# manuelbb-upb/Morbit.jl

Hardware: AMD Instinct MI355X
Metric: RBF build+solve+eval cycles/sec (higher is better)
Workload: dtype f64

## Files before the change

### include/mrbf.h

```cpp
#ifndef MRBF_H
#define MRBF_H

#include <stdint.h>

#ifdef __cplusplus
extern "C" {
#endif

typedef struct mrbf_ctx mrbf_ctx;
typedef struct mrbf_model mrbf_model;

enum {
    MRBF_CUBIC = 0,
    MRBF_INV_MULTIQUADRIC = 1,
    MRBF_MULTIQUADRIC = 2,
    MRBF_THIN_PLATE_SPLINE = 3,
    MRBF_GAUSSIAN = 4
};

enum {
    MRBF_OK = 0,
    MRBF_ENOTPD = 1,
    MRBF_ESINGULAR = 2,
    MRBF_EHIP = 3,
// ... 161 lines not shown
    const double *centres, *values;
    double *weights_out, *poly_out;
    mrbf_model *model;
    int32_t status;
    int32_t reserved;
    mrbf_fit_info info;
} mrbf_fit_job;
int32_t mrbf_fit_batch(mrbf_ctx *ctx, int64_t n_starts, mrbf_fit_job *jobs, float *ms_total);

int32_t mrbf_debug_env(const char *name);
int32_t mrbf_debug_mfma_layout(mrbf_ctx *ctx, double *out16x16_a_times_b, const double *A16x4, const double *B4x16);
int32_t mrbf_debug_potrf(mrbf_ctx *ctx, int64_t n, double *A_colmajor_inout, int32_t impl, int32_t *info, float *ms);
int32_t mrbf_debug_diag(mrbf_ctx *ctx, const double *A128, int32_t reps, float *ms_per_call, double *shader_cycles,
                        double *realtime_us);
int32_t mrbf_debug_mfma_peak(mrbf_ctx *ctx, int32_t blocks_per_cu, int32_t threads, int32_t iters, float *ms, double *tflops);
int32_t mrbf_debug_mfma_asm(mrbf_ctx *ctx, int32_t variant, int32_t blocks_per_cu, int32_t iters, float *ms, double *tflops,
                            double *cycles_per_mfma);
int32_t mrbf_debug_dgemm(mrbf_ctx *ctx, int32_t m, int32_t n, int32_t k, float *ms, double *tflops);
int32_t mrbf_debug_mega_tables(int32_t nt, int32_t mt, int32_t slack, int32_t slack_chain, int32_t first, int32_t win, int32_t srows,
                               int32_t half_cols, int64_t *out6);
int32_t mrbf_debug_mega_tables2(int32_t nt, int32_t mt, int32_t slack, int32_t slack_chain, int32_t first, int32_t win, int32_t srows,
                                int32_t half_cols, const int32_t *opt5, int64_t *out6);
int32_t mrbf_debug_mega_plan(int32_t nt, int32_t mt, int32_t xreal, int64_t *out39);

enum { MRBF_PS_OK = 0, MRBF_PS_CRITICAL = 1, MRBF_PS_FAILURE = 2 };
typedef struct {
    int32_t max_ideal_evals;
    int32_t max_ps_evals;
    int32_t max_polish_evals;
    int32_t reserved;
    uint64_t seed;
    double t0;
    double xtol_rel;
} mrbf_ps_options;
typedef struct {
    int32_t status;
    int32_t generations;
    int32_t evals_ideal, evals_ps, evals_polish;
    float ms_total;
    double tau;
} mrbf_ps_info;
int32_t mrbf_ps_step(mrbf_ctx *ctx, const mrbf_model *model, const double *x_n, const double *lb_eff, const double *ub_eff,
                     const double *fx_n, const double *r_or_null, const mrbf_ps_options *opts, double *x_trial, double *mx_trial,
                     double *r_out, mrbf_ps_info *info);

enum { MRBF_ROLE_NONE = -1, MRBF_ROLE_EQ = -2, MRBF_ROLE_INEQ = -3 };
// ... 120 lines not shown
```

### morbit.jl_amd/_lib.py

```python
import ctypes
import os

import numpy as np

_HERE = os.path.dirname(os.path.abspath(__file__))
LIB_PATH = os.environ.get("MRBF_LIB") or os.path.join(_HERE, "libmrbf.so")

c_dp = ctypes.POINTER(ctypes.c_double)
c_fp = ctypes.POINTER(ctypes.c_float)
c_ip = ctypes.POINTER(ctypes.c_int32)
c_vp = ctypes.c_void_p

MRBF_OK, MRBF_ENOTPD, MRBF_ESINGULAR, MRBF_EHIP, MRBF_EBLAS, MRBF_ENOMEM, MRBF_ENODEVICE, MRBF_ENCCL = range(8)
PATH_CHOL, PATH_PROJ_CHOL, PATH_LU, PATH_MINNORM, PATH_ROUND4 = 1, 2, 3, 4, 5
OPT_GRAM_MODE, OPT_RESIDUAL, OPT_FORCE_PATH, OPT_CHOL_IMPL, OPT_EVAL_IMPL, OPT_TIMING, OPT_DIAG_IMPL, OPT_CHOL_WINDOW = 1, 2, 3, 4, 5, 6, 7, 8
OPT_SPIN_MS, OPT_DEBUG_FAULT, OPT_LAST_DEVICE_MS, OPT_SLOW_LAUNCHES = 9, 10, 11, 12
OPT_ARENA_BYTES, OPT_LIVE_HANDLES = 13, 14
FB_CHOL_HOST_DRIVEN, FB_BACKSOLVE_BLOCKED, FB_LU = 1, 2, 4


class FitInfo(ctypes.Structure):
    _fields_ = [("path", ctypes.c_int32), ("factor_info", ctypes.c_int32), ("n", ctypes.c_int32), ("q", ctypes.c_int32),
                ("rel_residual", ctypes.c_double), ("max_pitw", ctypes.c_double), ("mu", ctypes.c_double),
                ("ms_gram", ctypes.c_float), ("ms_project", ctypes.c_float), ("ms_factor", ctypes.c_float),
# ... 158 lines not shown
                                     ctypes.c_double, ctypes.c_int32, ctypes.c_int32, ctypes.c_double, c_vp, c_ip, ctypes.POINTER(c_vp)]),
    "mrbf_fit_from_round4": (ctypes.c_int32, [c_vp, c_vp, ctypes.c_int32, c_vp, ctypes.POINTER(c_vp), c_vp, c_vp, ctypes.POINTER(FitInfo)]),
    "mrbf_round4_sites": (ctypes.c_int32, [c_vp, ctypes.POINTER(ctypes.c_int64), ctypes.POINTER(ctypes.c_int64), c_ip]),
    "mrbf_free_round4": (ctypes.c_int32, [c_vp, c_vp]),
    "mrbf_round4_batch": (ctypes.c_int32, [c_vp, ctypes.c_int64, ctypes.c_int32, ctypes.POINTER(Round4Job), c_fp]),
    "mrbf_dispatch_round4_batch": (ctypes.c_int32, [ctypes.c_int64, ctypes.c_int32]),
    "mrbf_model_dims": (ctypes.c_int32, [c_vp, ctypes.POINTER(ctypes.c_int64), c_ip, c_ip, c_ip]),
    "mrbf_free_model": (ctypes.c_int32, [c_vp, c_vp]),
    "mrbf_batch_run": (ctypes.c_int32, [ctypes.c_int32, c_ip, ctypes.c_int64, ctypes.POINTER(Problem),
                                        ctypes.POINTER(Result)]),
    "mrbf_fit_batch": (ctypes.c_int32, [c_vp, ctypes.c_int64, ctypes.POINTER(FitJob), c_fp]),
    "mrbf_dispatch_fit_batch": (ctypes.c_int32, [ctypes.c_int64]),
    "mrbf_debug_mfma_layout": (ctypes.c_int32, [c_vp, c_vp, c_vp, c_vp]),
    "mrbf_debug_potrf": (ctypes.c_int32, [c_vp, ctypes.c_int64, c_vp, ctypes.c_int32, c_ip, c_fp]),
    "mrbf_debug_env": (ctypes.c_int32, [ctypes.c_char_p]),
    "mrbf_debug_diag": (ctypes.c_int32, [c_vp, c_vp, ctypes.c_int32, c_fp, c_dp, c_dp]),
    "mrbf_debug_ps_rank": (ctypes.c_int32, [c_vp, ctypes.c_int32, c_vp, c_vp, ctypes.c_uint64, ctypes.c_int32, ctypes.c_int32, c_ip, c_ip]),
    "mrbf_debug_mfma_peak": (ctypes.c_int32, [c_vp, ctypes.c_int32, ctypes.c_int32, ctypes.c_int32, c_fp, c_dp]),
    "mrbf_debug_mfma_asm": (ctypes.c_int32, [c_vp, ctypes.c_int32, ctypes.c_int32, ctypes.c_int32, c_fp, c_dp, c_dp]),
    "mrbf_debug_dgemm": (ctypes.c_int32, [c_vp, ctypes.c_int32, ctypes.c_int32, ctypes.c_int32, c_fp, c_dp]),
    "mrbf_debug_mega_tables": (ctypes.c_int32, [ctypes.c_int32] * 8 + [c_vp]),
    "mrbf_debug_mega_tables2": (ctypes.c_int32, [ctypes.c_int32] * 8 + [c_vp, c_vp]),
    "mrbf_debug_mega_plan": (ctypes.c_int32, [ctypes.c_int32] * 3 + [c_vp]),
    "mrbf_stochastic_rank": (ctypes.c_int32, [ctypes.c_int32, c_vp, c_vp, c_vp, ctypes.c_double, c_vp]),
    "mrbf_ps_step": (ctypes.c_int32, [c_vp, c_vp, c_vp, c_vp, c_vp, c_vp, c_vp, ctypes.POINTER(PsOptions), c_vp, c_vp, c_vp,
                                      ctypes.POINTER(PsInfo)]),
    "mrbf_ps_step_problem": (ctypes.c_int32, [c_vp, ctypes.POINTER(PsProblem), c_vp, c_vp, c_vp, c_vp, c_vp, ctypes.POINTER(PsOptions),
                                              c_vp, c_vp, c_vp, ctypes.POINTER(PsInfo)]),
    "mrbf_sd_direction": (ctypes.c_int32, [c_vp, ctypes.c_int64, ctypes.c_int32, ctypes.c_int32, ctypes.c_int32, ctypes.c_int32] + [c_vp] * 8
                          + [ctypes.c_int32, c_vp, c_vp, c_vp, c_vp, c_vp]),
    "mrbf_sd_criticality": (ctypes.c_int32, [c_vp, ctypes.POINTER(PsProblem), c_vp, c_vp, c_vp, c_vp, ctypes.c_int32, c_vp, c_vp,
                                             ctypes.POINTER(SdInfo)]),
    "mrbf_normal_direction": (ctypes.c_int32, [c_vp, ctypes.c_int64, ctypes.c_int32, ctypes.c_int32, ctypes.c_int32] + [c_vp] * 12),
    "mrbf_normal_step": (ctypes.c_int32, [c_vp, ctypes.POINTER(PsProblem), ctypes.c_int32, c_vp, c_vp, c_vp, ctypes.c_double, ctypes.c_double,
                                          ctypes.c_double, ctypes.c_int32, c_vp, c_vp, ctypes.POINTER(NormalInfo)]),
    "mrbf_sd_step": (ctypes.c_int32, [c_vp, ctypes.POINTER(PsProblem), c_vp, c_vp, ctypes.c_double, c_vp, c_vp, ctypes.c_double, c_vp,
                                      ctypes.POINTER(SdStepOptions), c_vp, c_vp, ctypes.POINTER(SdStepInfo)]),
    "mrbf_sd_iterate_batch": (ctypes.c_int32, [c_vp, ctypes.c_int64, ctypes.POINTER(PsProblem), ctypes.POINTER(ctypes.c_void_p), c_vp, c_vp, c_vp,
                                               c_vp, c_vp, ctypes.c_int32, ctypes.POINTER(SdStepOptions), c_vp, c_vp, c_vp,
                                               ctypes.POINTER(SdBatchRecord), c_fp]),
    "mrbf_dispatch_sd_batch": (ctypes.c_int32, [ctypes.c_int64] + [ctypes.c_int32] * 7),
    "mrbf_normal_step_batch": (ctypes.c_int32, [c_vp, ctypes.c_int64, ctypes.POINTER(PsProblem), ctypes.POINTER(ctypes.c_void_p), ctypes.c_int32,
                                                c_vp, c_vp, c_vp, c_vp, ctypes.c_double, ctypes.c_double, ctypes.c_int32, c_vp, c_vp, c_vp,
                                                ctypes.POINTER(NormalBatchRecord), c_fp]),
    "mrbf_dispatch_normal_batch": (ctypes.c_int32, [ctypes.c_int64] + [ctypes.c_int32] * 5),
    "mrbf_dispatch_ps": (ctypes.c_int32, [ctypes.c_int32] * 6),
# ... 100 lines not shown
```

### morbit.jl_amd/csrc/chol_mega.hip

```cpp
#include <chrono>

#include "chol_diag_core.hpp"
#include "common.hpp"
#include "mega_gemm.hpp"

namespace mrbf {

typedef double v4d __attribute__((ext_vector_type(4)));
typedef double v2d __attribute__((ext_vector_type(2)));

namespace mega {

constexpr int WIN_DEFAULT = 4;

enum { JOB_U = 0, JOB_T = 1, JOB_P = 2, JOB_S = 3, JOB_UH = 4 };
struct Job {
    short kind, i, c, w;
};
enum { CTL_QP = 0, CTL_ABORT = 32, CTL_TIMEOUT = 64, CTL_PCOLS = 96, CTL_QC = 128, CTL_TS = 144 , CTL_WORDS = 160 };
constexpr int QSTRIDE = 32;
__host__ __device__ inline int wstart(int w, int first, int win) { return w <= 0 ? 0 : first + win * (w - 1); }
__host__ __device__ inline int nbulk_updates(int i, int c, int slack, int slack_chain, int first, int win, int srows = 2) {
    const int t = c - ((i - c <= srows) ? slack_chain : slack);
    return t < first ? 0 : (t - first) / win + 1;
// ... 24 lines not shown
    unsigned *sprog;
    unsigned *quiet;
    int nwin;
    int *info;
    const Job *cjobs;
    int nchainjobs;
    int nchain;
    int ndedicated;
    int look;
    unsigned long long spin_ticks;
    int fault;
    int use_quiet;
    int xchain;
    int quiet_tail;
    int slack, slack_chain, first, win, wbias, srows;
    Edge edge;
    int cboost;
    int head_job1;
    int nreserve;
    int reserve_job0;
    unsigned long long *jlog;
    int jlog_cap;
    int pstream;
    int panel_dma;
    int trace_dbg;
    unsigned long long *trace;
};

struct Shared {
    union {
        double gemm[4 * 2 * 8 * LDS_LD];
        diagcore::DiagV6Shared diag;
    } u;
    int ok;
    int jkind, jidx;
    unsigned long long *jrec;
    int wlo;
    int cwlo;
    int mycu;
};

typedef __attribute__((address_space(1))) unsigned gu32;
typedef __attribute__((address_space(1))) double gf64;
__device__ __forceinline__ unsigned ldf(const unsigned *p) {
    return __hip_atomic_load((const gu32 *)p, __ATOMIC_RELAXED, __HIP_MEMORY_SCOPE_AGENT);
}
// ... 155 lines not shown
                }
            }
        }
    }
}

template <int TM>
__device__ __forceinline__ void load_tile_neg(const double *__restrict__ C, int64_t ldc, v4d (&acc)[TM / 32][4]) {
    constexpr int NJ = TM / 32;
    const int lane = threadIdx.x & 63, wave = threadIdx.x >> 6;
    const int l15 = lane & 15, l4 = lane >> 4;
    const int ioff = (TM == 128) ? (wave >> 1) * 64 : 0;
    const int joff = (TM == 128) ? (wave & 1) * 64 : wave * 32;
#pragma unroll
    for (int j = 0; j < NJ; ++j)
#pragma unroll
        for (int r = 0; r < 4; ++r) {
            const int64_t gj = joff + j * 16 + l4 + 4 * r;
#pragma unroll
            for (int i = 0; i < 4; ++i) acc[j][i][r] = -*(const gf64 *)&C[(ioff + i * 16 + l15) + gj * ldc];
        }
}

#define JLOG(k)                                                             \
    do {                                                                   \
        if (sh.jrec && threadIdx.x == 0) sh.jrec[k] = wall_clock64();      \
    } while (0)

template <int TM>
__device__ __attribute__((noinline)) bool run_bulk(const Args &a, Shared &sh, const Job jb) {
    const int64_t lda = uni64(a.lda);
    double *const A = uni_ptr(a.A);
    const int i = __builtin_amdgcn_readfirstlane(jb.i), c = __builtin_amdgcn_readfirstlane(jb.c), jw = __builtin_amdgcn_readfirstlane(jb.w);
    const int w = jw & 255, hcode = jw >> 8, roff = (TM == 64 && hcode == 1) ? 64 : 0;
    const int pl = wstart(w + 1, a.first, a.win) - 1;
    if (!wg_wait(sh, a, a.tdone + (size_t)i * a.NT + pl, 2u, a.tdone + (size_t)c * a.NT + pl, 2u, a.ucnt + (size_t)i * a.NT + c,
                 (unsigned)(2 * w), 0x100u))
        return false;
    JLOG(2);
    v4d acc[TM / 32][4];
    double *C = A + (int64_t)i * NB + roff + (int64_t)c * NB * lda;
    load_tile_neg<TM>(C, lda, acc);
    const int64_t k0 = (int64_t)wstart(w, a.first, a.win) * NB;
    gemm_acc<TM>(A + (int64_t)i * NB + roff + k0 * lda, lda, A + (int64_t)c * NB + k0 * lda, lda,
                 (wstart(w + 1, a.first, a.win) - wstart(w, a.first, a.win)) * NB, acc, sh.u.gemm);
    JLOG(3);
#pragma unroll
    for (int j = 0; j < TM / 32; ++j)
#pragma unroll
        for (int i2 = 0; i2 < 4; ++i2) acc[j][i2] = -acc[j][i2];
    if (i == c)
        store_tile<TM, false, true, true>(C, lda, acc, roff);
    else
        store_tile<TM, false, false, true>(C, lda, acc);
    wg_drain();
    if (threadIdx.x == 0) addf(a.ucnt + (size_t)i * a.NT + c, (TM == 128 || hcode == 2) ? 2u : 1u);
    return true;
}

template <int TM>
__device__ __forceinline__ bool window_part(const Args &a, Shared &sh, int i, int c, int pend, int roff,
                                                      unsigned long long *tr) {
    const int64_t lda = uni64(a.lda);
    double *const A = uni_ptr(a.A);
    const int wc = nbulk_updates(i, c, a.slack, a.slack_chain, a.first, a.win, srows_at(c, a.srows, a.edge)), p0 = wstart(wc, a.first, a.win);
    const unsigned *uc = a.ucnt + (size_t)i * a.NT + c;
    if (p0 >= pend) return wg_wait(sh, a, uc, (unsigned)(2 * wc), nullptr, 0, nullptr, 0, 0x200u);
    v4d acc[TM / 32][4];
    zero_acc(acc);
    for (int p = p0; p < pend;) {
        if (threadIdx.x == 0) {
            bool ok = poll_ge(a.tdone + (size_t)i * a.NT + p, 2u, a, 0x210u) && poll_ge(a.tdone + (size_t)c * a.NT + p, 2u, a, 0x211u);
            int run = 0;
            if (ok) {
                run = 1;
                while (p + run < pend && ldf(a.tdone + (size_t)i * a.NT + p + run) >= 2u && ldf(a.tdone + (size_t)c * a.NT + p + run) >= 2u) ++run;
            }
            __builtin_amdgcn_fence(__ATOMIC_ACQUIRE, "agent");
            asm volatile("s_waitcnt vmcnt(0)" ::: "memory");
            sh.ok = run;
        }
        __syncthreads();
        const int run = sh.ok;
        __syncthreads();
        if (run == 0) return false;
        if (tr && threadIdx.x == 0) tr[p == p0 ? 5 : 6] = wall_clock64();
        JLOG(p == p0 ? 2 : 3);
        const int64_t k0 = (int64_t)p * NB;
        gemm_acc<TM>(A + (int64_t)i * NB + roff + k0 * lda, lda, A + (int64_t)c * NB + k0 * lda, lda, run * NB, acc, sh.u.gemm);
        p += run;
    }
    if (tr && threadIdx.x == 0) tr[7] = wall_clock64();
    if (!wg_wait(sh, a, uc, (unsigned)(2 * wc), nullptr, 0, nullptr, 0, 0x212u)) return false;
    double *C = A + (int64_t)i * NB + roff + (int64_t)c * NB * lda;
    if (TM == 128 && i == c)
        store_tile<TM, true, true, false>(C, lda, acc);
    else
        store_tile<TM, true, false, false>(C, lda, acc);
    asm volatile("s_waitcnt vmcnt(0)" ::: "memory");
    __syncthreads();
    return true;
}

template <bool HALF>
__device__ __attribute__((noinline)) bool run_stream(const Args &a, Shared &sh, const Job jb) {
    const int64_t lda = uni64(a.lda);
    double *const A = uni_ptr(a.A);
    const int i = __builtin_amdgcn_readfirstlane(jb.i), c = __builtin_amdgcn_readfirstlane(jb.c);
    const int hh = HALF ? __builtin_amdgcn_readfirstlane(jb.w) - 1 : 0, roff = 64 * hh;
    constexpr int RW = HALF ? 16 : 32, U = HALF ? 1 : 2;
    if (HALF ? !window_part<64>(a, sh, i, c, c > 0 ? c - 1 : 0, roff, nullptr) : !window_part<128>(a, sh, i, c, c > 0 ? c - 1 : 0, 0, nullptr)) return false;
    JLOG(4);
    const int lane = threadIdx.x & 63, wave = __builtin_amdgcn_readfirstlane(threadIdx.x >> 6);
    const int l15 = lane & 15, l4 = lane >> 4;
    double *C = A + (int64_t)i * NB + roff + (int64_t)c * NB * lda;
    const double *Lcc = A + (int64_t)c * NB + (int64_t)c * NB * lda;
    const double *itg = uni_ptr(a.itg + (size_t)c * 8 * 256);
    const unsigned *dprog = uni_ptr(a.dprog + (size_t)c * QSTRIDE);
// ... 128 lines not shown
                if (HALF)
                    addf(tdone_ic, 1u);
                else
                    stf(tdone_ic, 2u);
            }
            if (str) str[5] = wall_clock64();
        }
        __builtin_amdgcn_sched_barrier(0);
#pragma unroll
        for (int q = b + 2; q < 8; ++q)
#pragma unroll
            for (int u = 0; u < U; ++u)
#pragma unroll
                for (int s2 = 0; s2 < 4; ++s2) x[u][q] = __builtin_amdgcn_mfma_f64_16x16x4f64(-lq[q][s2], xs[u][s2], x[u][q], 0, 0, 0);
    }
    return true;
}

#define MEGA_STAMP(k)                                                          \
    do {                                                                       \
        if (tr && threadIdx.x == 0) tr[k] = wall_clock64();                    \
    } while (0)

template <bool TRACED>
__device__ __attribute__((noinline)) bool run_diag(const Args &a, Shared &sh, const Job jb) {
    const int64_t lda = uni64(a.lda);
    double *const A = uni_ptr(a.A);
    const int c = __builtin_amdgcn_readfirstlane(jb.c);
    unsigned long long *tr = TRACED ? a.trace + (size_t)(2 * c) * 8 : nullptr;
    MEGA_STAMP(0);
    const int pstream_c = edge_col(c, a.edge) ? a.edge.pstream_edge : a.pstream;
    const int pstream = c < pstream_c ? c : pstream_c;
    if (!window_part<128>(a, sh, c, c, c - pstream, 0, tr)) return false;
    MEGA_STAMP(1);
    JLOG(4);
    const int lane = threadIdx.x & 63, wave = __builtin_amdgcn_readfirstlane(threadIdx.x >> 6);
    const int l15 = lane & 15, l4 = lane >> 4;
    double *C = A + (int64_t)c * NB + (int64_t)c * NB * lda;
    double *Linv = a.linv + (size_t)c * NB * NB;
    diagcore::v4d acc[diagcore::NSLOT6];
    diagcore::diag_v6_load(C, lda, acc);
    {
        constexpr int PAN = 16 * LDS_LD;
        double *const ring = sh.u.gemm;
#pragma unroll 1
        for (int pp = c - pstream; pp < c; ++pp) {
            const double *Lp = A + (int64_t)c * NB + (int64_t)pp * NB * lda;
            const unsigned *sprog0 = uni_ptr(sprog_at(a, c - pp - 1, 0, pp)), *sprog1 = uni_ptr(sprog_at(a, c - pp - 1, 1, pp));
            auto issue_fold = [&](int b) {
                double *sl = ring + (b & 1) * PAN;
#pragma unroll
                for (int u = 0; u < 4; ++u) {
                    const int col = 4 * wave + u;
                    glds16(Lp + 2 * lane + (int64_t)(16 * b + col) * lda, sl + col * LDS_LD);
                }
            };
// ... 42 lines not shown
    JLOG(5);
    __builtin_amdgcn_s_setprio(3);
    const int bad = diagcore::diag_v6_core(C, lda, Linv, sh.u.diag, acc, a.itg + (size_t)c * 8 * 256, a.dprog + (size_t)c * QSTRIDE,
                                           TRACED ? tr + 15 : nullptr);
    __builtin_amdgcn_s_setprio(1);
    if (bad) {
        if (threadIdx.x == 0) {
            *(__attribute__((address_space(1))) int *)a.info = c * NB + bad;
            stf(a.ctl + CTL_ABORT, 1u);
        }
        return false;
    }
    MEGA_STAMP(3);
    JLOG(6);
    wg_drain();
    if (threadIdx.x == 0) {
        stf(a.tdone + (size_t)c * a.NT + c, 2u);
        addf(a.ctl + CTL_PCOLS, 1u);
    }
    MEGA_STAMP(4);
    return true;
}

template <bool FULL>
__device__ __attribute__((noinline)) bool run_panel(const Args &a, Shared &sh, const Job jb) {
    constexpr int TM = FULL ? 128 : 64;
    const int64_t lda = uni64(a.lda);
    double *const A = uni_ptr(a.A);
    const int i = __builtin_amdgcn_readfirstlane(jb.i), c = __builtin_amdgcn_readfirstlane(jb.c), wcode = __builtin_amdgcn_readfirstlane(jb.w);
    const int roff = (!FULL && wcode == 1) ? 64 : 0;
    if (!window_part<TM>(a, sh, i, c, c, roff, nullptr)) return false;
    JLOG(4);
    double *C = A + (int64_t)i * NB + roff + (int64_t)c * NB * lda;
    double *Linv = a.linv + (size_t)c * NB * NB;
    if (!wg_wait(sh, a, a.tdone + (size_t)c * a.NT + c, 2u, nullptr, 0, nullptr, 0, 0x300u)) return false;
    JLOG(5);
    v4d acc[TM / 32][4];
    zero_acc(acc);
    if (__builtin_amdgcn_readfirstlane(a.panel_dma))
        gemm_acc_v2<TM>(C, lda, Linv, NB, NB, acc, sh.u.gemm);
    else
        gemm_acc_v1<TM>(C, lda, Linv, NB, NB, acc, sh.u.gemm);
    store_tile<TM, false, false, true>(C, lda, acc);
    wg_drain();
    if (a.fault && i == a.MT - 1 && c == 0 && roff == 0) return true;
    if (threadIdx.x == 0) addf(a.tdone + (size_t)i * a.NT + c, (FULL || wcode == 3) ? 2u : 1u);
    return true;
}

__device__ __forceinline__ void jlog_begin(const Args &a, Shared &sh, const Job jb) {
    if (threadIdx.x == 0) {
        unsigned long long *r = nullptr;
        if (a.jlog) {
            const unsigned long long n = __hip_atomic_fetch_add((__attribute__((address_space(1))) unsigned long long *)a.jlog, 1ull,
                                                                __ATOMIC_RELAXED, __HIP_MEMORY_SCOPE_AGENT);
            if (n < (unsigned long long)a.jlog_cap) {
                r = a.jlog + 8 + n * 8;
                r[0] = (unsigned long long)(unsigned short)jb.kind | ((unsigned long long)(unsigned short)jb.i << 8) |
                       ((unsigned long long)(unsigned short)jb.c << 24) | ((unsigned long long)(unsigned short)jb.w << 40) |
                       ((unsigned long long)blockIdx.x << 52);
                r[1] = wall_clock64();
            }
        }
        sh.jrec = r;
    }
    __syncthreads();
// ... 107 lines not shown
                int idx = -1;
                if (!ldf(a.ctl + CTL_ABORT)) {
                    if (reserve) {
                        const unsigned qc = ldf(a.ctl + CTL_QC);
                        if (qc >= (unsigned)a.head_job1 && qc < (unsigned)a.reserve_job0) idx = -2;
                    }
                    if (idx != -2) {
                        const unsigned got = addf(a.ctl + CTL_QC, 1u);
                        if (got < (unsigned)a.nchainjobs) idx = (int)got;
                    }
                }
                sh.jidx = idx;
            }
            __syncthreads();
            const int idx = sh.jidx;
            __syncthreads();
            if (idx == -2) {
                leave = true;
                break;
            }
            if (idx < 0) break;
            const Job jb = a.cjobs[idx];
            jlog_begin(a, sh, jb);
            if (!(jb.kind == JOB_P ? (a.trace ? run_diag<true>(a, sh, jb) : run_diag<false>(a, sh, jb))
                                   : (jb.w == 0 ? run_stream<false>(a, sh, jb) : run_stream<true>(a, sh, jb))))
                break;
            jlog_end(sh);
        }
        if (a.use_quiet && threadIdx.x == 0) addf(myquiet, 0xffffffffu);
        if (!leave) return;
        __builtin_amdgcn_s_setprio(0);
        in_chain = false;
        idle_t0 = 0;
        nidle = 0;
        continue;
    }
    {
        if (threadIdx.x < 64) {
            int kind = -1, idx = 0;
            bool panel_left = false;
            if (ldf(a.ctl + CTL_ABORT)) {
                kind = -2;
            } else if (reserve && ldf(a.ctl + CTL_QC) >= (unsigned)a.reserve_job0 && ldf(a.ctl + CTL_QC) < (unsigned)a.nchainjobs) {
                kind = -3;
            } else if (!dedicated && a.use_quiet && ldf(myquiet) != 0 && a.NT - (int)ldf(a.ctl + CTL_PCOLS) <= a.quiet_tail) {
                kind = -1;
                idle_t0 = 0;
// ... 48 lines not shown
            }
        }
        __syncthreads();
        const int kind = sh.jkind, idx = sh.jidx;
        __syncthreads();
        if (kind == -2) break;
        if (kind == -3) {
            in_chain = true;
            continue;
        }
        if (kind == -1) {
            ++nidle;
            const int reps = nidle < 8 ? 1 : (nidle < 32 ? 4 : 16);
            for (int r = 0; r < reps; ++r) __builtin_amdgcn_s_sleep(64);
            continue;
        }
        idle_t0 = 0;
        nidle = 0;
        bool ok;
        const unsigned long long tj0 = a.trace ? wall_clock64() : 0ull;
        jlog_begin(a, sh, kind == 1 ? a.pjobs[idx] : a.bjobs[idx]);
        if (kind == 1) {
            if (!dedicated) __builtin_amdgcn_s_setprio(1);
            ok = a.pjobs[idx].w == 2 ? run_panel<true>(a, sh, a.pjobs[idx]) : run_panel<false>(a, sh, a.pjobs[idx]);
            if (!dedicated) __builtin_amdgcn_s_setprio(0);
        } else {
            ok = a.bjobs[idx].kind == JOB_UH ? run_bulk<64>(a, sh, a.bjobs[idx]) : run_bulk<128>(a, sh, a.bjobs[idx]);
        }
        jlog_end(sh);
        if (a.trace && threadIdx.x == 0) {
            unsigned long long *u = a.trace + (size_t)a.NT * 16 + (size_t)blockIdx.x * 4;
            u[kind == 1 ? 1 : 0] += wall_clock64() - tj0;
            u[kind == 1 ? 3 : 2] += 1;
        }
        if (!ok) break;
    }
    }
}

__global__ __launch_bounds__(256, 2) void potrf_mega_kernel(const Args a) {
    if (threadIdx.x == 0)
        __hip_atomic_fetch_max((unsigned long long *)(a.ctl + CTL_TS), ~(unsigned long long)wall_clock64(), __ATOMIC_RELAXED, __HIP_MEMORY_SCOPE_AGENT);
    mega_body(a);
    if (threadIdx.x == 0)
        __hip_atomic_fetch_max((unsigned long long *)(a.ctl + CTL_TS + 2), (unsigned long long)wall_clock64(), __ATOMIC_RELAXED, __HIP_MEMORY_SCOPE_AGENT);
}

__global__ void mega_status_kernel(const unsigned *ctl, int *info, unsigned long long *stat) {
    if (ctl[CTL_TIMEOUT] != 0 && *info == 0) *info = -(int)ctl[CTL_TIMEOUT];
    const unsigned long long *ts = (const unsigned long long *)(ctl + CTL_TS);
// ... 262 lines not shown
    a.wq_head = fl + CTL_WORDS;
    a.quiet = a.wq_head + (size_t)QSTRIDE * (2 * a.nwin + 1);
    a.dprog = a.quiet + (size_t)QSTRIDE * 512;
    a.sprog = a.dprog + (size_t)QSTRIDE * NT;
    a.tdone = a.sprog + (size_t)QSTRIDE * 2 * plan.srows_max * NT;
    a.ucnt = a.tdone + (size_t)MT * NT;
    a.info = dinfo;
    a.nchain = plan.nchain;
    a.ndedicated = plan.ndedicated;
    a.look = plan.look;
    a.use_quiet = plan.use_quiet;
    a.slack = tp.slack;
    a.slack_chain = tp.slack_chain;
    a.first = tp.first;
    a.win = tp.win;
    a.wbias = plan.wbias;
    a.srows = tp.srows;
    a.edge = tp.edge;
    a.cboost = plan.cboost;
    a.head_job1 = plan.head_job1;
    a.reserve_job0 = plan.reserve_job0;
    a.nreserve = plan.nreserve;
    a.panel_dma = plan.panel_dma;
    a.pstream = plan.pstream;
    a.xchain = plan.xchain;
    a.quiet_tail = plan.quiet_tail;
    a.spin_ticks = (unsigned long long)std::max(1, ctx->spin_ms) * 100000ull;
    a.fault = (ctx->debug_fault & 1) && MT > 1;
    const int grid = plan.grid;
    const char *trace_path = mrbf_env("MRBF_MEGA_TRACE");
    if (trace_path) {
        a.trace_dbg = mrbf_env("MRBF_MEGA_TRACE_WAVE") ? 12 + 16 * (atoi(mrbf_env("MRBF_MEGA_TRACE_WAVE")) & 3) : 4;
        MRBF_TRY(get_buf(ctx, S_MEGA_TRACE, (size_t)NT * 80 + 4 * 1024, &a.trace));
        MRBF_HIP(ctx, hipMemsetAsync(a.trace, 0, ((size_t)NT * 80 + 4 * 1024) * sizeof(unsigned long long), ctx->stream));
    }
    const char *jlog_path = mrbf_env("MRBF_MEGA_JLOG");
    if (jlog_path) {
        a.jlog_cap = a.npanel + a.nbulk + a.nchainjobs + 16;
        MRBF_TRY(get_buf(ctx, S_MEGA_JLOG, (size_t)8 * a.jlog_cap + 16, &a.jlog));
        MRBF_HIP(ctx, hipMemsetAsync(a.jlog, 0, ((size_t)8 * a.jlog_cap + 16) * sizeof(unsigned long long), ctx->stream));
    }
    hipLaunchKernelGGL(potrf_mega_kernel, dim3((unsigned)grid), dim3(256), 0, ctx->stream, a);
    hnow();
    if (jlog_path) {
        std::vector<unsigned long long> h((size_t)8 * a.jlog_cap + 16);
        MRBF_HIP(ctx, hipStreamSynchronize(ctx->stream));
// ... 178 lines not shown
    edge.tail_c0 = srows < edge.srows_edge ? std::max(edge.head, nt - opt5[1]) : nt;
    edge.shalf = (opt5[4] & 2) ? 1 : 0;
    edge.sh_head = (opt5[4] >> 2) & 0xff;
    edge.sh_tail_c0 = ((opt5[4] >> 10) & 0xff) ? std::max(edge.sh_head, nt - ((opt5[4] >> 10) & 0xff)) : (edge.sh_head ? nt : 0);
    edge.xhalf = (opt5[4] >> 26) & 1;
    edge.tfull1 = (opt5[4] >> 18) & 0xff;
    return check_mega_tables(nt, mt, mrbf::mega::TableParams{slack, slack_chain, first, win, srows, half_cols, opt5[2], opt5[3] > 0 ? opt5[3] : 1000, opt5[4] & 1, edge}, out);
}

extern "C" int32_t mrbf_debug_mega_plan(int32_t nt, int32_t mt, int32_t xreal, int64_t *out) {
    if (nt < 1 || mt < nt || mt > 32000) return -1;
    if (xreal < 0) return -3;
    if (!out) return -4;
    const mrbf::mega::Plan p = mrbf::mega::plan_for(nt, mt, mrbf::mega::Knobs{}, xreal);
    const mrbf::mega::TableParams &t = p.tp;
    const mrbf::mega::Edge &e = t.edge;
    const int v[33] = {t.slack, t.slack_chain, t.first, t.win, t.srows, t.half_cols, t.tail_half, t.tail_half_w, t.chainq,
                       e.head, e.tail_c0, e.srows_edge, e.pstream_edge, e.shalf, e.sh_head, e.sh_tail_c0, e.tfull1, e.xhalf,
                       p.nchain, p.ndedicated, p.nreserve, p.head_job1, p.reserve_job0, p.xchain, p.quiet_tail, p.pstream, p.look, p.use_quiet,
                       p.wbias, p.cboost, p.panel_dma, p.grid, p.srows_max};
    for (int i = 0; i < 33; ++i) out[i] = v[i];
    return check_mega_tables(nt, mt, t, out + 33);
}
```

### morbit.jl_amd/csrc/mega_gemm.hpp

```cpp
#pragma once
#include "common.hpp"

namespace mrbf {
namespace mega {

typedef double v4d __attribute__((ext_vector_type(4)));
typedef double v2d __attribute__((ext_vector_type(2)));
typedef __attribute__((address_space(1))) v2d gv2d;
constexpr int NB = 128, BK = 16, LDS_LD = NB + 16;

#ifndef MRBF_GEMM_NSTG
#define MRBF_GEMM_NSTG 4
#endif
#ifndef MRBF_GEMM_RAW_BARRIER
#define MRBF_RING_BARRIER() asm volatile("s_barrier" ::: "memory")
#else
#define MRBF_RING_BARRIER() __builtin_amdgcn_s_barrier()
#endif
constexpr int SK = 8, NSTG = MRBF_GEMM_NSTG;
constexpr int STG = 2 * SK * LDS_LD;
typedef __attribute__((address_space(3))) void lds_void;
typedef const __attribute__((address_space(1))) void glb_void;
__device__ __forceinline__ void glds16(const double *g, double *l) {
    __builtin_amdgcn_global_load_lds((glb_void *)g, (lds_void *)l, 16, 0, 0);
// ... 144 lines not shown
#pragma unroll
                    for (int i = 0; i < 4; ++i) av[i] = As[(kk * 4 + l4) * LDS_LD + ioff + i * 16 + l15];
#pragma unroll
                    for (int j = 0; j < NJ; ++j) bv[j] = Bs[(kk * 4 + l4) * LDS_LD + joff + j * 16 + l15];
#pragma unroll
                    for (int j = 0; j < NJ; ++j)
#pragma unroll
                        for (int i = 0; i < 4; ++i)
                            acc[j][i] = __builtin_amdgcn_mfma_f64_16x16x4f64(bv[j], av[i], acc[j][i], 0, 0, 0);
                }
            }
        }
    }
    __syncthreads();
}


template <int TM>
__device__ __forceinline__ void gemm_acc(const double *__restrict__ Ag, int64_t lda, const double *__restrict__ Bg, int64_t ldb, int K,
                                         v4d (&acc)[TM / 32][4], double *smem) {
    gemm_acc_v2<TM>(Ag, lda, Bg, ldb, K, acc, smem);
}

}
}
```

Measured before the change: 172.1.

## Skip upper-triangle MFMA work in diagonal SYRK, half-diagonal and triangular panel solves

Adds triangular-aware GEMM variants for the Cholesky megakernel. Diagonal 128x128 SYRK tiles use a balanced per-wave map that computes only the 36 lower 16x16 blocks (9 per wave). Half-diagonal bulk updates skip upper blocks, and panel solves against the triangular Linv truncate K per column block. This is enabled by default through MRBF_MEGA_TRI=3 and cuts MFMA and LDS work on the triangular tiles. In exchange it adds per-wave switch dispatch, more template instantiations (code size and register pressure), and new index maps that must be correct.

```diff
diff --git a/include/mrbf.h b/include/mrbf.h
--- a/include/mrbf.h
+++ b/include/mrbf.h
@@ -207,6 +207,7 @@
 int32_t mrbf_debug_mega_tables2(int32_t nt, int32_t mt, int32_t slack, int32_t slack_chain, int32_t first, int32_t win, int32_t srows,
                                 int32_t half_cols, const int32_t *opt5, int64_t *out6);
 int32_t mrbf_debug_mega_plan(int32_t nt, int32_t mt, int32_t xreal, int64_t *out39);
+int32_t mrbf_debug_tri_maps(int64_t *out14);
 
 enum { MRBF_PS_OK = 0, MRBF_PS_CRITICAL = 1, MRBF_PS_FAILURE = 2 };
 typedef struct {
diff --git a/morbit.jl_amd/_lib.py b/morbit.jl_amd/_lib.py
--- a/morbit.jl_amd/_lib.py
+++ b/morbit.jl_amd/_lib.py
@@ -204,6 +204,7 @@
     "mrbf_debug_mega_tables": (ctypes.c_int32, [ctypes.c_int32] * 8 + [c_vp]),
     "mrbf_debug_mega_tables2": (ctypes.c_int32, [ctypes.c_int32] * 8 + [c_vp, c_vp]),
     "mrbf_debug_mega_plan": (ctypes.c_int32, [ctypes.c_int32] * 3 + [c_vp]),
+    "mrbf_debug_tri_maps": (ctypes.c_int32, [c_vp]),
     "mrbf_stochastic_rank": (ctypes.c_int32, [ctypes.c_int32, c_vp, c_vp, c_vp, ctypes.c_double, c_vp]),
     "mrbf_ps_step": (ctypes.c_int32, [c_vp, c_vp, c_vp, c_vp, c_vp, c_vp, c_vp, ctypes.POINTER(PsOptions), c_vp, c_vp, c_vp,
                                       ctypes.POINTER(PsInfo)]),
diff --git a/morbit.jl_amd/csrc/chol_mega.hip b/morbit.jl_amd/csrc/chol_mega.hip
--- a/morbit.jl_amd/csrc/chol_mega.hip
+++ b/morbit.jl_amd/csrc/chol_mega.hip
@@ -70,6 +70,7 @@
     unsigned long long *jlog;
     int jlog_cap;
     int pstream;
+    int tri;
     int panel_dma;
     int trace_dbg;
     unsigned long long *trace;
@@ -271,12 +272,106 @@
         }
 }
 
+template <int TM, int KIND>
+__device__ __forceinline__ bool tri_block(int w, int j, int i, int &rb, int &cb) {
+    if constexpr (KIND == TRI_SYRK) {
+        const int s = j * 4 + i, r = s <= w ? 0 : 1;
+        cb = r == 0 ? s : s - (w + 1);
+        rb = tri::syrk_row(w, r);
+        return s < 9;
+    } else {
+        rb = ((TM == 128) ? (w >> 1) * 4 : 0) + i;
+        cb = tri::solve_col(TM, w, j);
+        return true;
+    }
+}
+template <int TM, int KIND, bool SUB, bool LOWER, bool SC1, class WV>
+__device__ __forceinline__ void store_tile_tri_w(WV wv, double *__restrict__ C, int64_t ldc, const v4d (&acc)[tri_nj<TM, KIND>()][4]) {
+    constexpr int NJ = tri_nj<TM, KIND>();
+    const int lane = threadIdx.x & 63, wave = wv.value;
+    const int l15 = lane & 15, l4 = lane >> 4;
+#pragma unroll
+    for (int j = 0; j < NJ; ++j) {
+        double cv[4][4];
+        if (SUB) {
+#pragma unroll
+            for (int i = 0; i < 4; ++i) {
+                int rb, cb;
+                if (tri_block<TM, KIND>(wave, j, i, rb, cb)) {
+#pragma unroll
+                    for (int r = 0; r < 4; ++r) cv[r][i] = *(const gf64 *)&C[(rb * 16 + l15) + (int64_t)(cb * 16 + l4 + 4 * r) * ldc];
+                }
+            }
+        }
+#pragma unroll
+        for (int i = 0; i < 4; ++i) {
+            int rb, cb;
+            if (tri_block<TM, KIND>(wave, j, i, rb, cb)) {
+#pragma unroll
+                for (int r = 0; r < 4; ++r) {
+                    const int64_t gi = rb * 16 + l15, gj = cb * 16 + l4 + 4 * r;
+                    const double v = SUB ? cv[r][i] - acc[j][i][r] : acc[j][i][r];
+                    if (!LOWER || gi >= gj) {
+                        if (SC1)
+                            st_sc1(C + gi + gj * ldc, v);
+                        else
+                            *(gf64 *)&C[gi + gj * ldc] = v;
+                    }
+                }
+            }
+        }
+    }
+}
+template <int TM, int KIND, class WV>
+__device__ __forceinline__ void load_tile_neg_tri_w(WV wv, const double *__restrict__ C, int64_t ldc, v4d (&acc)[tri_nj<TM, KIND>()][4]) {
+    constexpr int NJ = tri_nj<TM, KIND>();
+    const int lane = threadIdx.x & 63, wave = wv.value;
+    const int l15 = lane & 15, l4 = lane >> 4;
+#pragma unroll
+    for (int j = 0; j < NJ; ++j)
+#pragma unroll
+        for (int i = 0; i < 4; ++i) {
+            int rb, cb;
+            if (tri_block<TM, KIND>(wave, j, i, rb, cb)) {
+#pragma unroll
+                for (int r = 0; r < 4; ++r) acc[j][i][r] = -*(const gf64 *)&C[(rb * 16 + l15) + (int64_t)(cb * 16 + l4 + 4 * r) * ldc];
+            }
+        }
+}
+#define MRBF_TRI_WAVE_SWITCH(CALL)                               \
+    do {                                                         \
+        const int wave__ = __builtin_amdgcn_readfirstlane(threadIdx.x >> 6); \
+        if constexpr (KIND == TRI_SYRK) {                        \
+            switch (wave__) {                                    \
+                case 0: CALL(WaveC<0>{}); break;                 \
+                case 1: CALL(WaveC<1>{}); break;                 \
+                case 2: CALL(WaveC<2>{}); break;                 \
+                default: CALL(WaveC<3>{}); break;                \
+            }                                                    \
+        } else {                                                 \
+            CALL(WaveR{wave__});                                 \
+        }                                                        \
+    } while (0)
+template <int TM, int KIND, bool SUB, bool LOWER, bool SC1>
+__device__ __forceinline__ void store_tile_tri(double *__restrict__ C, int64_t ldc, const v4d (&acc)[tri_nj<TM, KIND>()][4]) {
+#define MRBF_CALL(WV) store_tile_tri_w<TM, KIND, SUB, LOWER, SC1>(WV, C, ldc, acc)
+    MRBF_TRI_WAVE_SWITCH(MRBF_CALL);
+#undef MRBF_CALL
+}
+template <int TM, int KIND>
+__device__ __forceinline__ void load_tile_neg_tri(const double *__restrict__ C, int64_t ldc, v4d (&acc)[tri_nj<TM, KIND>()][4]) {
+#define MRBF_CALL(WV) load_tile_neg_tri_w<TM, KIND>(WV, C, ldc, acc)
+    MRBF_TRI_WAVE_SWITCH(MRBF_CALL);
+#undef MRBF_CALL
+}
+#undef MRBF_TRI_WAVE_SWITCH
+
 #define JLOG(k)                                                             \
     do {                                                                   \
         if (sh.jrec && threadIdx.x == 0) sh.jrec[k] = wall_clock64();      \
     } while (0)
 
-template <int TM>
+template <int TM, bool TRI = false>
 __device__ __attribute__((noinline)) bool run_bulk(const Args &a, Shared &sh, const Job jb) {
     const int64_t lda = uni64(a.lda);
     double *const A = uni_ptr(a.A);
@@ -287,18 +382,31 @@
                  (unsigned)(2 * w), 0x100u))
         return false;
     JLOG(2);
-    v4d acc[TM / 32][4];
+    constexpr int NJ = (TRI && TM == 128) ? SYRK_NJ : TM / 32;
+    v4d acc[NJ][4];
     double *C = A + (int64_t)i * NB + roff + (int64_t)c * NB * lda;
-    load_tile_neg<TM>(C, lda, acc);
     const int64_t k0 = (int64_t)wstart(w, a.first, a.win) * NB;
-    gemm_acc<TM>(A + (int64_t)i * NB + roff + k0 * lda, lda, A + (int64_t)c * NB + k0 * lda, lda,
-                 (wstart(w + 1, a.first, a.win) - wstart(w, a.first, a.win)) * NB, acc, sh.u.gemm);
+    const double *Ai = A + (int64_t)i * NB + roff + k0 * lda, *Ac = A + (int64_t)c * NB + k0 * lda;
+    const int K = (wstart(w + 1, a.first, a.win) - wstart(w, a.first, a.win)) * NB;
+    if constexpr (TRI && TM == 128) {
+        zero_acc(acc);
+        load_tile_neg_tri<128, TRI_SYRK>(C, lda, acc);
+        gemm_acc_tri<128, TRI_SYRK>(Ai, lda, Ac, lda, K, acc, sh.u.gemm);
+    } else {
+        load_tile_neg<TM>(C, lda, acc);
+        if constexpr (TRI)
+            gemm_acc_tri<64, TRI_HALFDIAG>(Ai, lda, Ac, lda, K, acc, sh.u.gemm, roff);
+        else
+            gemm_acc<TM>(Ai, lda, Ac, lda, K, acc, sh.u.gemm);
+    }
     JLOG(3);
 #pragma unroll
-    for (int j = 0; j < TM / 32; ++j)
+    for (int j = 0; j < NJ; ++j)
 #pragma unroll
         for (int i2 = 0; i2 < 4; ++i2) acc[j][i2] = -acc[j][i2];
-    if (i == c)
+    if constexpr (TRI && TM == 128)
+        store_tile_tri<128, TRI_SYRK, false, true, true>(C, lda, acc);
+    else if (TRI || i == c)
         store_tile<TM, false, true, true>(C, lda, acc, roff);
     else
         store_tile<TM, false, false, true>(C, lda, acc);
@@ -307,15 +415,16 @@
     return true;
 }
 
-template <int TM>
+template <int TM, bool DIAG = false>
 __device__ __forceinline__ bool window_part(const Args &a, Shared &sh, int i, int c, int pend, int roff,
                                                       unsigned long long *tr) {
+    static_assert(!DIAG || TM == 128, "diagonal tiles are taken whole");
     const int64_t lda = uni64(a.lda);
     double *const A = uni_ptr(a.A);
     const int wc = nbulk_updates(i, c, a.slack, a.slack_chain, a.first, a.win, srows_at(c, a.srows, a.edge)), p0 = wstart(wc, a.first, a.win);
     const unsigned *uc = a.ucnt + (size_t)i * a.NT + c;
     if (p0 >= pend) return wg_wait(sh, a, uc, (unsigned)(2 * wc), nullptr, 0, nullptr, 0, 0x200u);
-    v4d acc[TM / 32][4];
+    v4d acc[DIAG ? SYRK_NJ : TM / 32][4];
     zero_acc(acc);
     for (int p = p0; p < pend;) {
         if (threadIdx.x == 0) {
@@ -336,13 +445,18 @@
         if (tr && threadIdx.x == 0) tr[p == p0 ? 5 : 6] = wall_clock64();
         JLOG(p == p0 ? 2 : 3);
         const int64_t k0 = (int64_t)p * NB;
-        gemm_acc<TM>(A + (int64_t)i * NB + roff + k0 * lda, lda, A + (int64_t)c * NB + k0 * lda, lda, run * NB, acc, sh.u.gemm);
+        if constexpr (DIAG)
+            gemm_acc_tri<128, TRI_SYRK>(A + (int64_t)i * NB + k0 * lda, lda, A + (int64_t)c * NB + k0 * lda, lda, run * NB, acc, sh.u.gemm);
+        else
+            gemm_acc<TM>(A + (int64_t)i * NB + roff + k0 * lda, lda, A + (int64_t)c * NB + k0 * lda, lda, run * NB, acc, sh.u.gemm);
         p += run;
     }
     if (tr && threadIdx.x == 0) tr[7] = wall_clock64();
     if (!wg_wait(sh, a, uc, (unsigned)(2 * wc), nullptr, 0, nullptr, 0, 0x212u)) return false;
     double *C = A + (int64_t)i * NB + roff + (int64_t)c * NB * lda;
-    if (TM == 128 && i == c)
+    if constexpr (DIAG)
+        store_tile_tri<128, TRI_SYRK, true, true, false>(C, lda, acc);
+    else if (TM == 128 && i == c)
         store_tile<TM, true, true, false>(C, lda, acc);
     else
         store_tile<TM, true, false, false>(C, lda, acc);
@@ -517,7 +631,7 @@
         if (tr && threadIdx.x == 0) tr[k] = wall_clock64();                    \
     } while (0)
 
-template <bool TRACED>
+template <bool TRACED, bool TRI>
 __device__ __attribute__((noinline)) bool run_diag(const Args &a, Shared &sh, const Job jb) {
     const int64_t lda = uni64(a.lda);
     double *const A = uni_ptr(a.A);
@@ -526,7 +640,7 @@
     MEGA_STAMP(0);
     const int pstream_c = edge_col(c, a.edge) ? a.edge.pstream_edge : a.pstream;
     const int pstream = c < pstream_c ? c : pstream_c;
-    if (!window_part<128>(a, sh, c, c, c - pstream, 0, tr)) return false;
+    if (!window_part<128, TRI>(a, sh, c, c, c - pstream, 0, tr)) return false;
     MEGA_STAMP(1);
     JLOG(4);
     const int lane = threadIdx.x & 63, wave = __builtin_amdgcn_readfirstlane(threadIdx.x >> 6);
@@ -615,7 +729,7 @@
     return true;
 }
 
-template <bool FULL>
+template <bool FULL, bool TRI>
 __device__ __attribute__((noinline)) bool run_panel(const Args &a, Shared &sh, const Job jb) {
     constexpr int TM = FULL ? 128 : 64;
     const int64_t lda = uni64(a.lda);
@@ -630,11 +744,16 @@
     JLOG(5);
     v4d acc[TM / 32][4];
     zero_acc(acc);
-    if (__builtin_amdgcn_readfirstlane(a.panel_dma))
-        gemm_acc_v2<TM>(C, lda, Linv, NB, NB, acc, sh.u.gemm);
-    else
-        gemm_acc_v1<TM>(C, lda, Linv, NB, NB, acc, sh.u.gemm);
-    store_tile<TM, false, false, true>(C, lda, acc);
+    if constexpr (TRI) {
+        gemm_acc_tri<TM, TRI_SOLVE>(C, lda, Linv, NB, NB, acc, sh.u.gemm);
+        store_tile_tri<TM, TRI_SOLVE, false, false, true>(C, lda, acc);
+    } else {
+        if (__builtin_amdgcn_readfirstlane(a.panel_dma))
+            gemm_acc_v2<TM>(C, lda, Linv, NB, NB, acc, sh.u.gemm);
+        else
+            gemm_acc_v1<TM>(C, lda, Linv, NB, NB, acc, sh.u.gemm);
+        store_tile<TM, false, false, true>(C, lda, acc);
+    }
     wg_drain();
     if (a.fault && i == a.MT - 1 && c == 0 && roff == 0) return true;
     if (threadIdx.x == 0) addf(a.tdone + (size_t)i * a.NT + c, (FULL || wcode == 3) ? 2u : 1u);
@@ -788,7 +907,9 @@
             if (idx < 0) break;
             const Job jb = a.cjobs[idx];
             jlog_begin(a, sh, jb);
-            if (!(jb.kind == JOB_P ? (a.trace ? run_diag<true>(a, sh, jb) : run_diag<false>(a, sh, jb))
+            const bool tri_diag = (a.tri & 1) != 0;
+            if (!(jb.kind == JOB_P ? (a.trace ? (tri_diag ? run_diag<true, true>(a, sh, jb) : run_diag<true, false>(a, sh, jb))
+                                              : (tri_diag ? run_diag<false, true>(a, sh, jb) : run_diag<false, false>(a, sh, jb)))
                                    : (jb.w == 0 ? run_stream<false>(a, sh, jb) : run_stream<true>(a, sh, jb))))
                 break;
             jlog_end(sh);
@@ -883,10 +1004,16 @@
         jlog_begin(a, sh, kind == 1 ? a.pjobs[idx] : a.bjobs[idx]);
         if (kind == 1) {
             if (!dedicated) __builtin_amdgcn_s_setprio(1);
-            ok = a.pjobs[idx].w == 2 ? run_panel<true>(a, sh, a.pjobs[idx]) : run_panel<false>(a, sh, a.pjobs[idx]);
+            const bool tri_solve = a.panel_dma && (a.tri & 2);
+            ok = a.pjobs[idx].w == 2 ? (tri_solve ? run_panel<true, true>(a, sh, a.pjobs[idx]) : run_panel<true, false>(a, sh, a.pjobs[idx]))
+                                     : (tri_solve ? run_panel<false, true>(a, sh, a.pjobs[idx]) : run_panel<false, false>(a, sh, a.pjobs[idx]));
             if (!dedicated) __builtin_amdgcn_s_setprio(0);
         } else {
-            ok = a.bjobs[idx].kind == JOB_UH ? run_bulk<64>(a, sh, a.bjobs[idx]) : run_bulk<128>(a, sh, a.bjobs[idx]);
+            const Job bj = a.bjobs[idx];
+            if ((a.tri & 1) && bj.i == bj.c)
+                ok = bj.kind == JOB_UH ? run_bulk<64, true>(a, sh, bj) : run_bulk<128, true>(a, sh, bj);
+            else
+                ok = bj.kind == JOB_UH ? run_bulk<64>(a, sh, bj) : run_bulk<128>(a, sh, bj);
         }
         jlog_end(sh);
         if (a.trace && threadIdx.x == 0) {
@@ -1195,6 +1322,7 @@
     a.reserve_job0 = plan.reserve_job0;
     a.nreserve = plan.nreserve;
     a.panel_dma = plan.panel_dma;
+    a.tri = mrbf_env("MRBF_MEGA_TRI") ? atoi(mrbf_env("MRBF_MEGA_TRI")) & 3 : 3;
     a.pstream = plan.pstream;
     a.xchain = plan.xchain;
     a.quiet_tail = plan.quiet_tail;
@@ -1419,3 +1547,8 @@
     for (int i = 0; i < 33; ++i) out[i] = v[i];
     return check_mega_tables(nt, mt, t, out + 33);
 }
+
+extern "C" int32_t mrbf_debug_tri_maps(int64_t *out14) {
+    if (!out14) return -100;
+    return mrbf::mega::tri::check_maps(out14);
+}
diff --git a/morbit.jl_amd/csrc/mega_gemm.hpp b/morbit.jl_amd/csrc/mega_gemm.hpp
--- a/morbit.jl_amd/csrc/mega_gemm.hpp
+++ b/morbit.jl_amd/csrc/mega_gemm.hpp
@@ -190,5 +190,277 @@
     gemm_acc_v2<TM>(Ag, lda, Bg, ldb, K, acc, smem);
 }
 
-}
-}
+namespace tri {
+constexpr int NBLK = NB / 16;
+__host__ __device__ constexpr int syrk_row(int w, int r) { return r == 0 ? w : NBLK - 1 - w; }
+__host__ __device__ constexpr bool syrk_owns(int w, int r, int jb) { return jb >= 0 && jb <= syrk_row(w, r); }
+__host__ __device__ constexpr int syrk_nblocks(int w) { return syrk_row(w, 0) + 1 + syrk_row(w, 1) + 1; }
+__host__ __device__ constexpr int syrk_nbfrag(int w) { return syrk_row(w, 1) + 1; }
+__host__ __device__ constexpr int syrk_slot(int w, int r, int jb) { return r == 0 ? jb : w + 1 + jb; }
+__host__ __device__ constexpr int solve_col(int tm, int w, int j) { return tm == 64 ? (j == 0 ? w : NBLK - 1 - w) : 4 * (w & 1) + j; }
+__host__ __device__ constexpr int solve_klim(int cb) { return 16 * (cb + 1); }
+__host__ __device__ constexpr bool half_keeps(int roff, int w, int j, int i) { return roff / 16 + i >= 2 * w + j; }
+
+inline int check_maps(int64_t *out) {
+    int rc = 0;
+    auto fail = [&](int code) {
+        if (rc == 0) rc = code;
+    };
+    int owners[NBLK][NBLK] = {};
+    for (int w = 0; w < 4; ++w) {
+        int nb = 0, slots[9] = {};
+        for (int r = 0; r < 2; ++r)
+            for (int jb = 0; jb < NBLK; ++jb)
+                if (syrk_owns(w, r, jb)) {
+                    ++nb;
+                    ++owners[syrk_row(w, r)][jb];
+                    if (syrk_slot(w, r, jb) < 0 || syrk_slot(w, r, jb) >= 9)
+                        fail(-1);
+                    else if (++slots[syrk_slot(w, r, jb)] != 1)
+                        fail(-1);
+                    if (jb >= syrk_nbfrag(w)) fail(-2);
+                }
+        out[w] = nb;
+        if (nb != 9 || nb != syrk_nblocks(w)) fail(-3);
+    }
+    int64_t lower = 0, upper = 0;
+    for (int ib = 0; ib < NBLK; ++ib)
+        for (int jb = 0; jb < NBLK; ++jb) {
+            if (jb <= ib) {
+                lower += owners[ib][jb];
+                if (owners[ib][jb] != 1) fail(-4);
+            } else {
+                upper += owners[ib][jb];
+                if (owners[ib][jb] != 0) fail(-5);
+            }
+        }
+    out[8] = lower;
+    out[9] = upper;
+    int colown[NBLK] = {};
+    for (int w = 0; w < 4; ++w) {
+        int kext = 0;
+        for (int j = 0; j < 2; ++j) {
+            const int cb = solve_col(64, w, j);
+            if (cb < 0 || cb >= NBLK) {
+                fail(-6);
+                continue;
+            }
+            ++colown[cb];
+            kext += solve_klim(cb);
+            if (solve_klim(cb) % 16 != 0 || solve_klim(cb) > NB) fail(-7);
+        }
+        out[4 + w] = kext;
+        if (kext != 144) fail(-8);
+        if (solve_klim(solve_col(64, w, 1)) < solve_klim(solve_col(64, w, 0))) fail(-9);
+    }
+    int64_t covered = 0;
+    for (int cb = 0; cb < NBLK; ++cb) {
+        covered += colown[cb];
+        if (colown[cb] != 1) fail(-10);
+    }
+    out[10] = covered;
+    int colown128[NBLK] = {};
+    for (int w = 0; w < 4; ++w)
+        for (int j = 0; j < 4; ++j) {
+            const int cb = solve_col(128, w, j);
+            if (cb < 0 || cb >= NBLK) {
+                fail(-11);
+                continue;
+            }
+            ++colown128[cb];
+            if (j > 0 && solve_col(128, w, j) < solve_col(128, w, j - 1)) fail(-12);
+        }
+    for (int cb = 0; cb < NBLK; ++cb)
+        if (colown128[cb] != 2) fail(-13);
+    int64_t beyond = 0;
+    for (int j = 0; j < NB; ++j)
+        for (int k = 0; k <= j; ++k)
+            if (k >= solve_klim(j / 16)) ++beyond;
+    out[11] = beyond;
+    if (beyond != 0) fail(-14);
+    int keep[NBLK][NBLK] = {};
+    for (int roff = 0; roff < NB; roff += 64)
+        for (int w = 0; w < 4; ++w)
+            for (int j = 0; j < 2; ++j)
+                for (int i = 0; i < 4; ++i)
+                    if (half_keeps(roff, w, j, i)) ++keep[roff / 16 + i][2 * w + j];
+    int64_t hl = 0, hu = 0;
+    for (int ib = 0; ib < NBLK; ++ib)
+        for (int jb = 0; jb < NBLK; ++jb) {
+            if (jb <= ib) {
+                hl += keep[ib][jb];
+                if (keep[ib][jb] != 1) fail(-15);
+            } else {
+                hu += keep[ib][jb];
+                if (keep[ib][jb] != 0) fail(-16);
+            }
+        }
+    out[12] = hl;
+    out[13] = hu;
+    return rc;
+}
+}
+
+enum { TRI_SYRK = 0, TRI_SOLVE = 1, TRI_HALFDIAG = 2 };
+constexpr int SYRK_NJ = 3;
+template <int TM, int KIND>
+constexpr int tri_nj() {
+    return KIND == TRI_SYRK ? SYRK_NJ : TM / 32;
+}
+template <int W>
+struct WaveC {
+    static constexpr int value = W;
+};
+struct WaveR {
+    int value;
+};
+
+template <int TM, int KIND>
+__device__ __forceinline__ void gemm_acc_tri(const double *__restrict__ Ag, int64_t lda, const double *__restrict__ Bg, int64_t ldb, int K,
+                                             v4d (&acc)[tri_nj<TM, KIND>()][4], double *smem, int roff = 0) {
+    static_assert(KIND != TRI_SYRK || TM == 128, "the balanced map of a diagonal tile is for 128 rows");
+    static_assert(KIND != TRI_HALFDIAG || TM == 64, "halves of a diagonal tile have 64 rows");
+    constexpr int NJ = TM / 32;
+    constexpr int NFB = KIND == TRI_SYRK ? tri::NBLK : NJ;
+    constexpr bool WSWITCH = !(KIND == TRI_SOLVE && TM == 128);
+    const int tid = threadIdx.x, lane = tid & 63, wave = __builtin_amdgcn_readfirstlane(tid >> 6);
+    const int l15 = lane & 15, l4 = lane >> 4;
+    const int nst = __builtin_amdgcn_readfirstlane(K / SK);
+    const int rblk = __builtin_amdgcn_readfirstlane(roff >> 4);
+    const double *ap = Ag + (int64_t)(2 * wave) * lda + 2 * ((TM == 128) ? lane : (lane & 31));
+    const double *bp = Bg + (int64_t)(2 * wave) * ldb + 2 * lane;
+    auto issue = [&](int st) {
+        double *sA = smem + (st % NSTG) * STG + 2 * wave * LDS_LD;
+        double *sB = sA + SK * LDS_LD;
+        const double *ga = ap + (int64_t)st * SK * lda;
+        const double *gb = bp + (int64_t)st * SK * ldb;
+        glds16(ga, sA);
+        glds16(ga + lda, sA + LDS_LD);
+        glds16(gb, sB);
+        glds16(gb + ldb, sB + LDS_LD);
+    };
+    auto frag = [&](auto wc, int st, int kk, double (&av)[4], double (&bv)[NFB]) {
+        const int W = wc.value;
+        const double *sA = smem + (st % NSTG) * STG + (kk * 4 + l4) * LDS_LD;
+        const double *sB = sA + SK * LDS_LD;
+        if constexpr (KIND == TRI_SYRK) {
+#pragma unroll
+            for (int r = 0; r < 2; ++r) av[r] = sA[tri::syrk_row(W, r) * 16 + l15];
+#pragma unroll
+            for (int jb = 0; jb < tri::NBLK; ++jb)
+                if (jb < tri::syrk_nbfrag(W)) bv[jb] = sB[jb * 16 + l15];
+        } else if constexpr (KIND == TRI_SOLVE) {
+            const int ioff = (TM == 128) ? (W >> 1) * 64 : 0;
+            if (st * SK < tri::solve_klim(tri::solve_col(TM, W, NJ - 1))) {
+#pragma unroll
+                for (int i = 0; i < 4; ++i) av[i] = sA[ioff + i * 16 + l15];
+            }
+#pragma unroll
+            for (int j = 0; j < NJ; ++j)
+                if (st * SK < tri::solve_klim(tri::solve_col(TM, W, j))) bv[j] = sB[tri::solve_col(TM, W, j) * 16 + l15];
+        } else {
+#pragma unroll
+            for (int i = 0; i < 4; ++i) av[i] = sA[i * 16 + l15];
+#pragma unroll
+            for (int j = 0; j < NJ; ++j) bv[j] = sB[W * 32 + j * 16 + l15];
+        }
+    };
+    auto mma = [&](auto wc, int st, const double (&av)[4], const double (&bv)[NFB], int part) {
+        const int W = wc.value;
+        if constexpr (KIND == TRI_SYRK) {
+#pragma unroll
+            for (int jb = 0; jb < tri::NBLK; ++jb)
+                if ((jb < 2) == (part == 0)) {
+#pragma unroll
+                    for (int r = 0; r < 2; ++r)
+                        if (tri::syrk_owns(W, r, jb))
+                            acc[tri::syrk_slot(W, r, jb) >> 2][tri::syrk_slot(W, r, jb) & 3] = __builtin_amdgcn_mfma_f64_16x16x4f64(
+                                bv[jb], av[r], acc[tri::syrk_slot(W, r, jb) >> 2][tri::syrk_slot(W, r, jb) & 3], 0, 0, 0);
+                }
+        } else if constexpr (KIND == TRI_SOLVE) {
+#pragma unroll
+            for (int j = 0; j < NJ; ++j)
+                if ((j < 1) == (part == 0)) {
+                    if (st * SK < tri::solve_klim(tri::solve_col(TM, W, j))) {
+#pragma unroll
+                        for (int i = 0; i < 4; ++i) acc[j][i] = __builtin_amdgcn_mfma_f64_16x16x4f64(bv[j], av[i], acc[j][i], 0, 0, 0);
+                    }
+                }
+        } else {
+#pragma unroll
+            for (int j = 0; j < NJ; ++j)
+                if ((j < 1) == (part == 0)) {
+#pragma unroll
+                    for (int i = 0; i < 4; ++i)
+                        if (rblk + i >= 2 * W + j) acc[j][i] = __builtin_amdgcn_mfma_f64_16x16x4f64(bv[j], av[i], acc[j][i], 0, 0, 0);
+                }
+        }
+    };
+    const int npro = nst < NSTG ? nst : NSTG;
+    for (int st = 0; st < npro; ++st) issue(st);
+    wait_stages(npro - 1);
+    asm volatile("s_waitcnt lgkmcnt(0)" ::: "memory");
+    MRBF_RING_BARRIER();
+    double xa[4], xb[NFB], ya[4], yb[NFB];
+#define MRBF_TRI_HALF_W(WC, FA, FB, ST, RD, RST, RKK, NA, NBF) \
+    {                                                          \
+        mma(WC, ST, FA, FB, 0);                                \
+        __builtin_amdgcn_sched_barrier(0);                     \
+        if (RD) frag(WC, RST, RKK, NA, NBF);                   \
+        __builtin_amdgcn_sched_barrier(0);                     \
+        mma(WC, ST, FA, FB, 1);                                \
+        __builtin_amdgcn_sched_barrier(0);                     \
+    }
+#define MRBF_TRI_HALF(FA, FB, ST, RD, RST, RKK, NA, NBF)                                      \
+    if constexpr (!WSWITCH) {                                                                 \
+        MRBF_TRI_HALF_W(WaveR{wave}, FA, FB, ST, RD, RST, RKK, NA, NBF)                       \
+    } else {                                                                                  \
+        switch (wave) {                                                                       \
+            case 0: MRBF_TRI_HALF_W(WaveC<0>{}, FA, FB, ST, RD, RST, RKK, NA, NBF) break;     \
+            case 1: MRBF_TRI_HALF_W(WaveC<1>{}, FA, FB, ST, RD, RST, RKK, NA, NBF) break;     \
+            case 2: MRBF_TRI_HALF_W(WaveC<2>{}, FA, FB, ST, RD, RST, RKK, NA, NBF) break;     \
+            default: MRBF_TRI_HALF_W(WaveC<3>{}, FA, FB, ST, RD, RST, RKK, NA, NBF) break;    \
+        }                                                                                     \
+    }
+    if constexpr (!WSWITCH) {
+        frag(WaveR{wave}, 0, 0, xa, xb);
+    } else {
+        switch (wave) {
+            case 0: frag(WaveC<0>{}, 0, 0, xa, xb); break;
+            case 1: frag(WaveC<1>{}, 0, 0, xa, xb); break;
+            case 2: frag(WaveC<2>{}, 0, 0, xa, xb); break;
+            default: frag(WaveC<3>{}, 0, 0, xa, xb); break;
+        }
+    }
+    int st = 0;
+#pragma unroll 1
+    for (; st + NSTG < nst; ++st) {
+        MRBF_TRI_HALF(xa, xb, st, true, st, 1, ya, yb);
+        if constexpr (NSTG == 4)
+            asm volatile("s_waitcnt vmcnt(8)" ::: "memory");
+        else
+            asm volatile("s_waitcnt vmcnt(4)" ::: "memory");
+        asm volatile("s_waitcnt lgkmcnt(0)" ::: "memory");
+        MRBF_RING_BARRIER();
+        issue(st + NSTG);
+        __builtin_amdgcn_sched_barrier(0);
+        MRBF_TRI_HALF(ya, yb, st, true, st + 1, 0, xa, xb);
+    }
+#pragma unroll 1
+    for (; st + 1 < nst; ++st) {
+        MRBF_TRI_HALF(xa, xb, st, true, st, 1, ya, yb);
+        wait_stages(nst - 2 - st);
+        asm volatile("s_waitcnt lgkmcnt(0)" ::: "memory");
+        MRBF_RING_BARRIER();
+        __builtin_amdgcn_sched_barrier(0);
+        MRBF_TRI_HALF(ya, yb, st, true, st + 1, 0, xa, xb);
+    }
+    MRBF_TRI_HALF(xa, xb, st, true, st, 1, ya, yb);
+    MRBF_TRI_HALF(ya, yb, st, false, st, 1, xa, xb);
+#undef MRBF_TRI_HALF
+#undef MRBF_TRI_HALF_W
+    __syncthreads();
+}
+
+}
+}
```

Measured after the change: 166.6. 3.2% lower.
